# ruotianluo/ImageCaptioning.pytorch

Hardware: AMD Instinct MI355X
Metric: captions/sec/node (UpDown SCST, bs10xsample_n5, 36x2048 feats) (higher is better)
Workload: dtype f32; 1 GPU; UpDown SCST (BASELINE configs[2]): per-GPU batch 10 x train_sample_n 5, 36x2048 bottom-up feats, R=E=1000 A=512, vocab 9487, seq_len 20, references packed+cooked + greedy baseline + CIDEr-D + RewardCriterion + BPTT + clip 0.1 + Adam; rotating_batches=4, global_batch=10, seq_len=20, parallelism=dp1 (flat fp32 gradient, no collective)

## Files before the change

imagecaptioning/pytorch_amd/_lib.py:

```python
import ctypes as C
import os

import torch

HERE = os.path.dirname(os.path.abspath(__file__))
LIB_PATH = os.environ.get('CAPMI_LIB') or os.path.join(HERE, 'libcapmi.so')
MAX_SEG = 4
MAX_BCOL = 3
EINVAL = -1

c_f = C.c_void_p


class GemmSeg(C.Structure):
    _fields_ = [('A', c_f), ('B', c_f), ('lda', C.c_int), ('ldb', C.c_int), ('K', C.c_int), ('a_row_div', C.c_int)]


class GemmDesc(C.Structure):
    _fields_ = [('seg', GemmSeg * MAX_SEG), ('nseg', C.c_int), ('a_layout', C.c_int), ('b_layout', C.c_int),
                ('M', C.c_int), ('N', C.c_int), ('C', c_f), ('ldc', C.c_int), ('bias', c_f), ('bias2', c_f),
                ('row_bias', c_f), ('row_bias_div', C.c_int), ('mul_mask', c_f), ('relu', C.c_int),
                ('accumulate', C.c_int), ('partial', c_f), ('partial_capacity', C.c_int64), ('splits', C.c_int),
                ('defer_reduce', C.c_int), ('splits_used', C.c_int), ('a_planes', c_f * MAX_SEG), ('addend', c_f),
                ('allow_wide_deferred', C.c_int), ('n_bcol', C.c_int), ('bcol_B', c_f * MAX_BCOL), ('bcol_ldb', C.c_int * MAX_BCOL),
# ... 5 lines not shown
                ('alive', c_f)]


class UpDownWeights(C.Structure):
    _fields_ = [(k, c_f) for k in (
        'embed', 'att_w_ih', 'att_w_hh', 'att_b_ih', 'att_b_hh', 'lang_w_ih', 'lang_w_hh', 'lang_b_ih', 'lang_b_hh',
        'h2att_w', 'h2att_b', 'alpha_w', 'alpha_b', 'logit_w', 'logit_b')]


class UpDownRollout(C.Structure):
    _fields_ = ([(k, C.c_int) for k in ('B', 'n', 'N', 'K', 'A', 'R', 'E', 'V1', 'B_feat')] + [('row_img', c_f)] +
                [(k, C.c_int) for k in ('T', 'L')] +
                [(k, c_f) for k in ('fc', 'att', 'p_att', 'att_mask', 'drop_xt', 'drop_out')] +
                [('mode', C.c_int), ('row_mode', c_f), ('temperature', C.c_float), ('gumbel', c_f),
                 ('seed', C.c_uint64), ('forced', c_f), ('forced_ld', C.c_int), ('teacher', C.c_int)] +
                [(k, c_f) for k in ('h_att', 'c_att', 'h_lang', 'c_lang', 'xt', 'it_all', 'gates_att', 'gates_lang',
                                    'att_h', 'alpha', 'ctx', 'h_drop', 'seq', 'seq_logp', 'sel_logp', 'live',
                                    'fc_gates', 'logits', 'it', 'unfinished', 'partial')] +
                [('partial_capacity', C.c_int64), ('top_k', C.c_int), ('top_p', C.c_float), ('ss_mode', c_f),
                 ('planes', c_f), ('planes_bytes', C.c_int64), ('early_exit', C.c_int), ('early_exit_from', C.c_int),
                 ('alive_host', c_f), ('steps_run', C.c_int), ('pre_partial', c_f), ('pre_capacity', C.c_int64), ('raw_logits', C.c_int)])


class SampleFilter(C.Structure):
    _fields_ = [('top_k', C.c_int), ('top_p', C.c_float)]


class UpDownGrads(C.Structure):
    _fields_ = [(k, c_f) for k in (
        'embed', 'att_w_ih', 'att_w_hh', 'att_b_ih', 'att_b_hh', 'lang_w_ih', 'lang_w_hh', 'lang_b_ih', 'lang_b_hh',
        'h2att_w', 'h2att_b', 'alpha_w', 'alpha_b', 'logit_w', 'logit_b', 'd_fc', 'd_att', 'd_p_att')]


class SparseLogpGrad(C.Structure):
    _fields_ = [('g_sel', c_f), ('g_sum', c_f), ('tok', c_f), ('tok_ld', C.c_int), ('raw', C.c_int), ('scale', c_f)]


class MaskDesc(C.Structure):
    _fields_ = [('mask', c_f), ('count', C.c_int64), ('offset', C.c_uint64), ('row_len', C.c_int), ('rows', C.c_int),
                ('keep_from', C.c_int)]


class ReduceItem(C.Structure):
    _fields_ = [('partial', c_f), ('C', c_f), ('bias', c_f), ('splits', C.c_int32), ('M', C.c_int32), ('N', C.c_int32),
                ('ldc', C.c_int32), ('accumulate', C.c_int32), ('reserved', C.c_int32)]

# ... 124 lines not shown

class Ensemble(C.Structure):
    _fields_ = ([(k, C.c_int) for k in ('M', 'rows', 'V1', 'ld_in', 'ld_out')] + [('in', c_f * ENSEMBLE_MAX),
                ('w', C.c_float * ENSEMBLE_MAX), ('out', c_f)])


class Ppo(C.Structure):
    _fields_ = ([(k, C.c_int) for k in ('N', 'L', 'V1', 'n', 'ld_new', 'ld_old', 'ld_grad', 'per_row')] +
                [('eps', C.c_float), ('kl_coef', C.c_float)] +
                [(k, c_f) for k in ('lp_new', 'lp_old', 'seq', 'scores', 'row_stats', 'msum', 'out', 'loss_rows', 'g_out', 'grad')])


_I, _F, _P, _U64, _I64 = C.c_int, C.c_float, C.c_void_p, C.c_uint64, C.c_int64
DECODE_NO_REPEAT, DECODE_NO_BAD_ENDING, DECODE_BLOCK_TRIGRAMS = 1, 2, 4
SELECT_RAW = 256

SIGNATURES = {
    'capmi_version': [],
    'capmi_arch': [],
    'capmi_gemm_f32': [C.POINTER(GemmDesc), _P],
    'capmi_planes_bytes': [_I],
    'capmi_planes_from_f32': [_P, _I, _I, _I, _P, _P],
    'capmi_updown_planes_bytes': [_I, _I],
    'capmi_updown_bwd_planes_bytes': [_I],
    'capmi_attention_fwd': [_P] * 8 + [_I] * 5 + [_P, _I, _P],
    'capmi_attention_fwd_partial': [_P, _I, _I64, _P, _P] + [_P] * 7 + [_I] * 5 + [_P, _I, _P],
    'capmi_attention_fwd_partial_pl': [_P, _I, _I64, _P, _P] + [_P] * 7 + [_I] * 5 + [_P, _I, _P, _P],
    'capmi_attention_bwd': [_P, _I] + [_P] * 8 + [_I] * 5 + [_P, _I, _P],
    'capmi_attention_bwd_partial': [_P, _I, _I64, _I, _P] + [_P] * 7 + [_I] * 5 + [_P, _I, _P],
    'capmi_attention_bwd_batched': [_P, _I] + [_P] * 9 + [_I] * 7 + [_P],
    'capmi_attention_bwd_batched_ws': [_P, _I] + [_P] * 9 + [_I] * 7 + [_P, _P],
    'capmi_lstm_cell_fwd': [_P, _I, _P, _P, _P, _I, _P] + [_P] * 6 + [_I, _I, _P],
    'capmi_lstm_cell_fwd_pl': [_P, _I, _P, _P, _P, _I, _P] + [_P] * 6 + [_I, _I, _P, _P, _P],
    'capmi_lstm_cell_fwd_pl2': [_P, _I, _P, _I, _P, _P, _P, _I, _P] + [_P] * 6 + [_I, _I, _P, _P, _P],
    'capmi_lstm_cell_bwd': [_P, _I, _P, _P, _I, _P, _I] + [_P] * 6 + [_I, _I, _P],
    'capmi_lstm_cell_bwd_partial_pl': [_P, _I, _P, _P, _I, _I, _I64, _P, _I, _I, _I64] + [_P] * 6 + [_I, _I, _P, _P],
    'capmi_embed_fwd_pl': [_P, _I, _P, _P, _P, _P, _I, _I, _I, _P, _P],
    'capmi_lstm_cell_bwd_partial': [_P, _I, _P, _P, _I, _I, _I64, _P, _I, _I, _I64] + [_P] * 6 + [_I, _I, _P],
    'capmi_embed_fwd': [_P, _I, _P, _P, _P, _P, _I, _I, _I, _P],
    'capmi_embed_bwd': [_P] * 5 + [_I, _I, _I, _P],
    'capmi_logsoftmax_select': [_P, _I, _I, _I, _I, _I, _P, _F, _P, _U64, _P, _I, _I, _P, _I, _P, _P, _P, _P, _P, _P],
    'capmi_logsoftmax_select_partial': [_P, _I, _I64, _P, _I, _I, _I, _I, _I, _P, _F, _P, _U64, _P, _I, _I, _P, _I, _P, _P, _P,
                                        _P, _P, _P, _P, _P],
    'capmi_logsoftmax_select_partial_gemm': [_P, _I, _I64, _P, _I, _I, _I, _I, _I, _P, _F, _P, _U64, _P, _I, _I, _P, _I, _P, _P, _P,
                                        _P, _P, _P, _P, _P, _P],
    'capmi_logsoftmax_bwd': [_P, _P, _P, _P, _I, _I, _I, _I, _P],
# ... 135 lines not shown
```

imagecaptioning/pytorch_amd/captioning/models/AttModel.py:

```python
import torch
import torch.nn as nn

from .CaptionModel import CaptionModel
from imagecaptioning.pytorch_amd import updown_engine as engine
from imagecaptioning.pytorch_amd import ops
from imagecaptioning.pytorch_amd import sparse_logp
from imagecaptioning.pytorch_amd._lib import CapmiError

from .utils import parse_sample_method, clip_len


class _RolloutFn(torch.autograd.Function):

    @staticmethod
    def forward(ctx, model, cfg, fc_feats, att_feats, att_masks, *params):
        P = dict(zip(model._param_names, [p.detach() for p in params]))
        if cfg.get('fused_greedy'):
            B = fc_feats.shape[0]
            K = clip_len(att_masks, att_feats.shape[1])
            R, A = P['fc_embed.0.weight'].shape[0], P['ctx2att.weight'].shape[0]
            dev = fc_feats.device
            pr_run = engine.Prepared()
            pr_run.fc = torch.empty(2 * B, R, dtype=torch.float32, device=dev)
            pr_run.att = torch.empty(2 * B, K, R, dtype=torch.float32, device=dev)
            pr_run.p_att = torch.empty(2 * B, K, A, dtype=torch.float32, device=dev)
            pr = engine.prepare(P, fc_feats, att_feats, att_masks, cfg.get('drop_fc'), cfg.get('drop_att'),
                                out=(pr_run.fc[:B], pr_run.att[:B], pr_run.p_att[:B]))
            engine.prepare(P, fc_feats, att_feats, att_masks, out=(pr_run.fc[B:], pr_run.att[B:], pr_run.p_att[B:]))
            pr_run.att_masks = None if pr.att_masks is None else torch.cat([pr.att_masks, pr.att_masks], 0)
            extra = dict(row_img=cfg['row_img'], B_grad=B)
        else:
            pr = engine.prepare(P, fc_feats, att_feats, att_masks, cfg.get('drop_fc'), cfg.get('drop_att'))
            pr_run, extra = pr, {}
        ro = engine.Rollout(P, pr_run, n=cfg['n'], T=cfg['T'], L=cfg['L'], mode=cfg['mode'],
                            temperature=cfg.get('temperature', 1.0), drop_xt=cfg.get('drop_xt'),
                            drop_out=cfg.get('drop_out'), gumbel=cfg.get('gumbel'), seed=cfg.get('seed', 0),
                            forced=cfg.get('forced'), teacher=cfg.get('teacher', False), row_mode=cfg.get('row_mode'),
                            top_k=cfg.get('top_k', 0), top_p=cfg.get('top_p', 0.0), ss_mode=cfg.get('ss_mode'),
                            raw_logits=cfg.get('raw_logits', False), **extra)
        seq, seq_logp = ro.run()
        ctx.model, ctx.ro, ctx.pr, ctx.P = model, ro, pr, P
        ctx.sink = sink = cfg.get('_sink')
        if sink is not None:
            sink.sel, sink.seq = ro.sel_logp, ro.seq
        ctx.set_materialize_grads(False)
        ctx.mark_non_differentiable(seq)
        model._last_rollout = ro
        return seq, seq_logp.detach()

    @staticmethod
    def backward(ctx, _g_seq, g_logp):
        model, ro, pr, P = ctx.model, ctx.ro, ctx.pr, ctx.P
# ... 259 lines not shown
```

imagecaptioning/pytorch_amd/csrc/gemm_f32.hip:

```cpp
#include "host_common.h"
#include "profile.h"
#include "gemm_common.h"
#include <atomic>
#include <stdio.h>
#include <stdlib.h>
#include <hip/hip_ext.h>

using namespace capmi_gemm;

namespace {

template <int ROWS, bool KC>
__device__ __forceinline__ void g2r(f32x4 (&r)[ROWS * BK / 4 / NT], const float *__restrict__ src, int ld,
                                    int row0, int nrows, int k0, int K, int row_div, int vec) {
    constexpr int NV = ROWS * BK / 4 / NT;
#pragma unroll
    for (int p = 0; p < NV; ++p) {
        const int idx = p * NT + threadIdx.x;
        f32x4 v = {0.f, 0.f, 0.f, 0.f};
        if (KC) {
            const int rr = idx / (BK / 4);
            const int kq = (idx % (BK / 4)) * 4;
            const int row = row0 + rr;
            const int k = k0 + kq;
// ... 203 lines not shown
            for (int s0 = 0; s0 < a.splits; s0 += 8) {
                float tv[8];
#pragma unroll
                for (int u = 0; u < 8; ++u) tv[u] = (s0 + u < a.splits) ? pp[(size_t)(s0 + u) * MN] : 0.f;
#pragma unroll
                for (int u = 0; u < 8; ++u) v += tv[u];
            }
            if (a.bias) v += a.bias[col];
            if (a.bias2) v += a.bias2[col];
            if (a.row_bias) v += a.row_bias[(size_t)(row / a.row_bias_div) * a.N + col];
            if (a.relu) v = fmaxf(v, 0.f);
            if (a.mul_mask) v *= a.mul_mask[(size_t)row * a.N + col];
            if (a.accumulate) v += a.addend[(size_t)row * a.ldc + col];
            a.C[(size_t)row * a.ldc + col] = v;
        }
    }
    if (threadIdx.x == 0) __hip_atomic_store(ticket, 0, __ATOMIC_RELAXED, __HIP_MEMORY_SCOPE_AGENT);
}

template <bool VEC>
__global__ void splitk_reduce_kernel(const float *__restrict__ partial, int splits, float *__restrict__ C, int ldc,
                                     int M, int N, const float *bias, const float *bias2, const float *row_bias,
                                     int row_bias_div, const float *mul_mask, int relu, int accumulate,
                                     const float *__restrict__ addend) {
    const size_t total = (size_t)M * N;
    if (VEC) {
        const unsigned quads = (unsigned)(total >> 2), nq = (unsigned)N >> 2;
        for (unsigned q = blockIdx.x * blockDim.x + threadIdx.x; q < quads; q += gridDim.x * blockDim.x) {
            const unsigned row = q / nq, col = (q - row * nq) * 4;
            const size_t i = (size_t)q * 4;
            f32x4 v = {0.f, 0.f, 0.f, 0.f};
            for (int s0 = 0; s0 < splits; s0 += 8) {
                f32x4 tv[8];
#pragma unroll
                for (int u = 0; u < 8; ++u)
                    tv[u] = (s0 + u < splits) ? *reinterpret_cast<const f32x4 *>(partial + (size_t)(s0 + u) * total + i) : f32x4{0.f, 0.f, 0.f, 0.f};
#pragma unroll
                for (int u = 0; u < 8; ++u) v += tv[u];
            }
            if (bias) v += *reinterpret_cast<const f32x4 *>(bias + col);
            if (bias2) v += *reinterpret_cast<const f32x4 *>(bias2 + col);
            if (row_bias) v += *reinterpret_cast<const f32x4 *>(row_bias + (size_t)(row / row_bias_div) * N + col);
            if (relu) { v[0] = fmaxf(v[0], 0.f); v[1] = fmaxf(v[1], 0.f); v[2] = fmaxf(v[2], 0.f); v[3] = fmaxf(v[3], 0.f); }
            if (mul_mask) v *= *reinterpret_cast<const f32x4 *>(mul_mask + i);
            if (accumulate) v += *reinterpret_cast<const f32x4 *>(addend + (size_t)row * ldc + col);
            *reinterpret_cast<f32x4 *>(C + (size_t)row * ldc + col) = v;
        }
        return;
    }
    for (size_t i = (size_t)blockIdx.x * blockDim.x + threadIdx.x; i < total; i += (size_t)gridDim.x * blockDim.x) {
        const int row = (int)(i / N), col = (int)(i % N);
        float v = 0.f;
        for (int s0 = 0; s0 < splits; s0 += 8) {
            float tv[8];
#pragma unroll
            for (int u = 0; u < 8; ++u) tv[u] = (s0 + u < splits) ? partial[(size_t)(s0 + u) * total + i] : 0.f;
#pragma unroll
            for (int u = 0; u < 8; ++u) v += tv[u];
        }
        if (bias) v += bias[col];
        if (bias2) v += bias2[col];
        if (row_bias) v += row_bias[(size_t)(row / row_bias_div) * N + col];
        if (relu) v = fmaxf(v, 0.f);
        if (mul_mask) v *= mul_mask[i];
        float *o = C + (size_t)row * ldc + col;
        if (accumulate) v += addend[(size_t)row * ldc + col];
        *o = v;
    }
}

__global__ __launch_bounds__(256) void splitk_reduce_batch_kernel(const capmi_reduce_item *__restrict__ items) {
    const capmi_reduce_item it = items[blockIdx.y];
    const size_t total = (size_t)it.M * it.N;
    const bool vec = it.N % 4 == 0 && it.ldc % 4 == 0 && ((reinterpret_cast<uintptr_t>(it.partial) | reinterpret_cast<uintptr_t>(it.C)) & 15) == 0 &&
                     (!it.bias || (reinterpret_cast<uintptr_t>(it.bias) & 15) == 0);
    if (vec) {
        const size_t quads = total / 4;
        for (size_t q = (size_t)blockIdx.x * blockDim.x + threadIdx.x; q < quads; q += (size_t)gridDim.x * blockDim.x) {
            const size_t i = q * 4;
            const int row = (int)(i / it.N), col = (int)(i % it.N);
            f32x4 v = {0.f, 0.f, 0.f, 0.f};
            for (int s0 = 0; s0 < it.splits; s0 += 4) {
                f32x4 tv[4];
#pragma unroll
                for (int u = 0; u < 4; ++u)
                    tv[u] = (s0 + u < it.splits) ? *reinterpret_cast<const f32x4 *>(it.partial + (size_t)(s0 + u) * total + i)
// ... 24 lines not shown
};
template <typename K>
void launch_one(K kernel, dim3 grid, hipStream_t st, const KArgs &a, const ProfInfo &pi) {
    hipEvent_t e0, e1;
    if (capmi_prof::take_events(pi.cls, &e0, &e1, pi.bytes, pi.flops))
        hipExtLaunchKernelGGL(kernel, grid, dim3(NT), 0, st, e0, e1, 0, a);
    else
        hipLaunchKernelGGL(kernel, grid, dim3(NT), 0, st, a);
}
template <int BM, int BN, int WM, int WN, int PF>
int launch_cfg(const KArgs &a, int al, int bl, dim3 grid, hipStream_t st, const ProfInfo &pi) {
    if (al == 0 && bl == 0) launch_one(gemm_kernel<BM, BN, WM, WN, true, true, PF>, grid, st, a, pi);
    else if (al == 0 && bl == 1) launch_one(gemm_kernel<BM, BN, WM, WN, true, false, PF>, grid, st, a, pi);
    else if (al == 1 && bl == 1) launch_one(gemm_kernel<BM, BN, WM, WN, false, false, PF>, grid, st, a, pi);
    else launch_one(gemm_kernel<BM, BN, WM, WN, false, true, PF>, grid, st, a, pi);
    CAPMI_CHECK_LAUNCH();
    return 0;
}

}

static int splitk_reduce_addend(const float *partial, int splits, float *C, int ldc, int M, int N, const float *bias, const float *bias2,
                                const float *row_bias, int row_bias_div, const float *mul_mask, int relu, int accumulate,
                                const float *addend, void *stream) {
    if (!partial || !C || splits < 1 || M <= 0 || N <= 0) return CAPMI_EINVAL;
    const size_t total = (size_t)M * N;
    const float *ad = addend ? addend : C;
    const bool vec = N % 4 == 0 && ldc % 4 == 0 && total < (1ull << 32) &&
                     ((reinterpret_cast<uintptr_t>(partial) | reinterpret_cast<uintptr_t>(C) | reinterpret_cast<uintptr_t>(bias) |
                       reinterpret_cast<uintptr_t>(bias2) | reinterpret_cast<uintptr_t>(row_bias) | reinterpret_cast<uintptr_t>(mul_mask) |
                       reinterpret_cast<uintptr_t>(ad)) & 15) == 0;
    const size_t work = vec ? total / 4 : total;
    int blocks = (int)((work + 255) / 256);
    if (blocks > 2048) blocks = 2048;
    if (vec)
        hipLaunchKernelGGL(splitk_reduce_kernel<true>, dim3(blocks), dim3(256), 0, (hipStream_t)stream, partial, splits, C, ldc, M, N, bias,
                           bias2, row_bias, row_bias_div > 0 ? row_bias_div : 1, mul_mask, relu, accumulate, ad);
    else
        hipLaunchKernelGGL(splitk_reduce_kernel<false>, dim3(blocks), dim3(256), 0, (hipStream_t)stream, partial, splits, C, ldc, M, N, bias,
                           bias2, row_bias, row_bias_div > 0 ? row_bias_div : 1, mul_mask, relu, accumulate, ad);
    CAPMI_CHECK_LAUNCH();
    return 0;
}

extern "C" int capmi_splitk_reduce(const float *partial, int splits, float *C, int ldc, int M, int N,
                                   const float *bias, const float *bias2, const float *row_bias, int row_bias_div,
                                   const float *mul_mask, int relu, int accumulate, void *stream) {
    return splitk_reduce_addend(partial, splits, C, ldc, M, N, bias, bias2, row_bias, row_bias_div, mul_mask, relu, accumulate, nullptr,
                                stream);
}

extern "C" int capmi_splitk_reduce_batch(const capmi_reduce_item *items, int n_items, void *stream) {
    if (!items || n_items <= 0) return CAPMI_EINVAL;
    hipLaunchKernelGGL(splitk_reduce_batch_kernel, dim3(64, n_items), dim3(256), 0, (hipStream_t)stream, items);
    CAPMI_CHECK_LAUNCH();
    return 0;
}

static std::atomic<int> g_wide_deferred{0};

extern "C" int capmi_gemm_set_policy(int allow_wide_deferred) {
    return g_wide_deferred.exchange(allow_wide_deferred ? 1 : 0);
}

extern "C" int capmi_gemm_f32(capmi_gemm_desc *d, void *stream) {
    if (!d || d->nseg < 1 || d->nseg > CAPMI_MAX_SEG || d->M <= 0 || d->N <= 0 || !d->C) return CAPMI_EINVAL;
    if (d->a_layout < 0 || d->a_layout > 1 || d->b_layout < 0 || d->b_layout > 1) return CAPMI_EINVAL;
    KArgs a{};
    a.nseg = d->nseg;
    static_assert(CAPMI_MAX_BCOL == MAX_BCOL, "column segments of the descriptor and of the kernel arguments");
    if (d->n_bcol < 0 || d->n_bcol > MAX_BCOL) return CAPMI_EINVAL;
    if (d->n_bcol > 0) {
        if (d->nseg != 1 || d->b_layout != 1) return CAPMI_EINVAL;
        int ncol = 0, blk = 0;
        for (int i = 0; i < d->n_bcol; ++i) {
            if (!d->bcol_B[i] || d->bcol_n[i] <= 0 || d->bcol_n[i] % 4 || d->bcol_ldb[i] % 4 || d->bcol_ldb[i] < d->bcol_n[i] ||
                !aligned16(d->bcol_B[i]))
                return CAPMI_EINVAL;
            a.bcol[i] = BCol{d->bcol_B[i], d->bcol_ldb[i], d->bcol_n[i], blk, ncol};
            ncol += d->bcol_n[i];
            blk += (d->bcol_n[i] + 127) / 128;
        }
        if (ncol != d->N) return CAPMI_EINVAL;
        a.nbcol = d->n_bcol;
    }
    int tiles = 0;
    for (int s = 0; s < d->nseg; ++s) {
        capmi_gemm_seg g = d->seg[s];
        if (a.nbcol) { g.B = a.bcol[0].B; g.ldb = a.bcol[0].ldb; }
        if (g.K <= 0) return CAPMI_EINVAL;
// ... 18 lines not shown
    a.ablate = env_ablate;
    a.M = d->M; a.N = d->N; a.C = d->C; a.ldc = d->ldc;
    a.bias = d->bias; a.bias2 = d->bias2; a.row_bias = d->row_bias;
    a.row_bias_div = d->row_bias_div > 0 ? d->row_bias_div : 1;
    a.mul_mask = d->mul_mask; a.relu = d->relu; a.accumulate = d->accumulate;
    a.addend = d->addend ? d->addend : d->C;
    const int64_t slab_cap = d->partial ? d->partial_capacity - CAPMI_WS_COUNTER_FLOATS : 0;
    a.partial = d->partial ? d->partial + CAPMI_WS_COUNTER_FLOATS : nullptr;
    a.counters = reinterpret_cast<int *>(d->partial);
    hipStream_t st = (hipStream_t)stream;
    double ksum = 0, abytes = 0;
    for (int s = 0; s < d->nseg; ++s) {
        ksum += d->seg[s].K;
        abytes += (double)d->seg[s].K * ((double)d->M / a.seg[s].a_row_div);
    }
    const double bytes = 4.0 * (abytes + ksum * d->N + (double)d->M * d->N);
    const double flops = 2.0 * d->M * (double)d->N * ksum;
    int pcls = (d->M <= 64 && d->a_layout == 0) ? (d->b_layout == 0 ? CAPMI_PROF_GEMM_DECODE : CAPMI_PROF_GEMM_BPTT)
                                                 : CAPMI_PROF_GEMM_FAT;
    if (pcls == CAPMI_PROF_GEMM_DECODE && bytes >= 24e6) pcls = CAPMI_PROF_GEMM_DECODE_STREAM;

    static const int env_path = capmi::research("CAPMI_GEMM_PATH", 0);
    static const int env_blocks = capmi::research("CAPMI_GEMM_BLOCKS", 512);
    bool ares_ok = d->a_layout == 0 && d->M <= 64 && BK == 32;
    for (int s = 0; s < d->nseg && ares_ok; ++s)
        ares_ok = a.seg[s].vecA && (a.seg[s].K % 4 == 0) && (d->b_layout == 1 || a.seg[s].vecB);
    static const int env_lc = capmi::knob("CAPMI_LC", 1);
    {
        bool lc_ok = env_lc && env_path != 3 && ares_ok && d->M <= 64;
        for (int s = 0; s < d->nseg && lc_ok; ++s)
            lc_ok = d->a_planes[s] != nullptr && a.seg[s].a_row_div == 1 && a.seg[s].vecB;
        if (lc_ok && d->b_layout == 1) lc_ok = d->N % 4 == 0 && d->N >= 4;
        if (lc_ok) {
            static const int env_ab = capmi::research("CAPMI_ARES_BLOCKS", 256);
            static const int env_opt = capmi::research("CAPMI_LC_OPT", 1);
            const int want = d->splits > 0 ? ((d->N + 127) / 128) * d->splits : env_ab;
            int splits = 0;
            a.sl = lc_plan(d->N, tiles, want, &splits);
            const bool partial = splits > 1 || d->defer_reduce;
            if (!partial || (d->partial && (int64_t)splits * d->M * d->N <= slab_cap)) {
                a.splits = splits;
                a.to_partial = partial ? 1 : 0;
                a.self_reduce = 0;
                a.ablate = env_opt;
                d->splits_used = splits;
                int rc = launch_lc(a, d->b_layout, st, pcls, bytes, flops);
                if (rc) return rc;
                if (splits > 1 && !d->defer_reduce)
                    return splitk_reduce_addend(a.partial, splits, d->C, d->ldc, d->M, d->N, d->bias, d->bias2, d->row_bias,
                                               a.row_bias_div, d->mul_mask, d->relu, d->accumulate, d->addend, stream);
                return 0;
            }
        }
    }
    if (a.nbcol) return CAPMI_EINVAL;
    if (env_path != 3 && ares_ok) {
        static const int env_ab = capmi::research("CAPMI_ARES_BLOCKS", 256);
        static const int env_ax3 = capmi::knob("CAPMI_ARES_X3", 1);
        int use_x3 = env_ax3;
        const int want = d->splits > 0 ? ((d->N + 127) / 128) * d->splits : env_ab;
        int splits = 0;
        int ts_cap = ares_ts_cap(d->M, use_x3);
        int ts_max = ares_plan(d->N, tiles, want, ts_cap, &splits);
        if (use_x3 && ((d->N + 127) / 128) * splits > want) {
            const int nblk = (d->N + 127) / 128;
            int splits2 = 0;
            const int ts2 = ares_plan(d->N, tiles, 2 * want, 3, &splits2);
            if (nblk * splits2 <= 2 * want && (int64_t)splits2 * d->M * d->N <= slab_cap) {
                ts_cap = 3; ts_max = ts2; splits = splits2;
            } else {
                int splits32 = 0;
                const int ts32 = ares_plan(d->N, tiles, want, ares_ts_cap(d->M, 0), &splits32);
                if (nblk * splits32 <= want) {
                    use_x3 = 0; ts_cap = ares_ts_cap(d->M, 0); ts_max = ts32; splits = splits32;
                }
            }
        }
        if ((splits > 1 || d->defer_reduce) && (int64_t)splits * d->M * d->N > slab_cap) ts_max = 99;
        if (ts_max <= ts_cap) {
            a.splits = splits;
            a.to_partial = (splits > 1 || d->defer_reduce) ? 1 : 0;
            a.self_reduce = 0;
            static const int env_aopt = capmi::research("CAPMI_ARES_OPT", 2);
            a.ablate = env_aopt;
            if (a.to_partial && (!d->partial || (int64_t)splits * d->M * d->N > slab_cap)) return CAPMI_EINVAL;
            d->splits_used = splits;
            int rc = launch_ares(a, d->b_layout, ts_max, use_x3, st, pcls, bytes, flops);
            if (rc) return rc;
            if (splits > 1 && !d->defer_reduce)
                return splitk_reduce_addend(a.partial, splits, d->C, d->ldc, d->M, d->N, d->bias, d->bias2, d->row_bias,
                                           a.row_bias_div, d->mul_mask, d->relu, d->accumulate, d->addend, stream);
            return 0;
        }
    }

    static const int env_cfg = capmi::research("CAPMI_GEMM_CFG", 1);
    int BM, BN;
    (void)env_cfg;
    if (d->M <= 32) { BM = 32; BN = 128; }
    else if (d->M <= 64 || (long long)d->M * d->N < 256LL * 1024) {
        BM = 64;
        BN = (d->b_layout == 0 && tiles >= 64 && d->N >= 1024) ? 128 : 64;
        if (env_cfg == 64 || env_cfg == 128) BN = env_cfg;
    } else { BM = 128; BN = 128; }
    const int gm = (d->M + BM - 1) / BM, gn = (d->N + BN - 1) / BN;
    static const int env_x3 = capmi::knob("CAPMI_GEMM_X3", 1);
    bool x3_ok = env_x3 && BM == 128 && BN == 128 && BK == 32 &&
                 (d->a_layout == 0 || d->M % 4 == 0) && (d->b_layout == 0 || d->N % 4 == 0);
    for (int s = 0; s < d->nseg && x3_ok; ++s)
        x3_ok = a.seg[s].a_row_div == 1 && a.seg[s].vecA && a.seg[s].vecB && a.seg[s].K % 4 == 0 &&
                (uint64_t)(d->a_layout == 0 ? d->M : 1) * (uint64_t)a.seg[s].lda * 4 < (1ull << 32) &&
                (uint64_t)(d->b_layout == 0 ? d->N : 1) * (uint64_t)a.seg[s].ldb * 4 < (1ull << 32);
    int splits = d->splits;
    static const int env_tile = capmi::knob("CAPMI_X3_TILE", 0);
    static const int env_wcost = capmi::research("CAPMI_X3W_COST", 165);
    static const int env_swap = capmi::knob("CAPMI_X3_SWAP", 1);
    int tiling = 0;
    const int gmw = (d->M + 255) / 256, gnw = (d->N + 255) / 256;
    if (x3_ok) {
        double best = 1e30;
        int best_sp = 1;
        const int sp_lo = splits > 0 ? splits : 1, sp_hi = splits > 0 ? splits : 16;
        for (int w = 0; w < 3; ++w) {
            if ((w == 0 && env_tile == 256) || (w >= 1 && env_tile == 128)) continue;
            if (w == 1 && env_tile != 256 && gmw < 4) continue;
            if (w == 1 && env_tile != 256 && d->defer_reduce && !d->allow_wide_deferred && !g_wide_deferred.load(std::memory_order_relaxed)) continue;
            if (w == 2 && (env_swap == 0 || d->a_layout != 0 || gnw < 4 || gmw >= 4)) continue;
            const int out_tiles = w == 0 ? gm * gn : w == 1 ? gmw * gn : gnw * gm;
            const double step = w ? env_wcost / 100.0 : 1.0;
            for (int sp = sp_lo; sp <= sp_hi && sp <= tiles; ++sp) {
                if (splits == 0 && sp > 1 && (!d->partial || (int64_t)sp * d->M * d->N > slab_cap)) break;
                const double rounds = (double)((out_tiles * sp + 255) / 256);
                const double slab_us = sp > 1 ? (2.0 * sp + 1.0) * d->M * (double)d->N * 4.0 / 4.0e6 : 0.0;
                const double cost = rounds * ((tiles + sp - 1) / sp) * step + slab_us / 1.5;
                if (cost < best) { best = cost; best_sp = sp; tiling = w; }
            }
        }
        if (splits == 0) splits = best_sp;
    } else if (splits == 0) {
        const int blocks = gm * gn;
        splits = 1;
        if (blocks < env_blocks * 3 / 4 && d->partial) {
            splits = (env_blocks + blocks - 1) / blocks;
            if (splits > tiles / 4) splits = tiles / 4;
            if (splits > 64) splits = 64;
            if (splits < 1) splits = 1;
            while (splits > 1 && (int64_t)splits * d->M * d->N > slab_cap) --splits;
        }
    }
    if (splits > tiles) splits = tiles;
    a.splits = splits;
    a.to_partial = (splits > 1 || d->defer_reduce) ? 1 : 0;
    static const int env_self = capmi::research("CAPMI_GEMM_SELF_REDUCE", 0);
    a.self_reduce = (env_self && splits > 1 && !d->defer_reduce && gn * gm <= CAPMI_WS_COUNTER_FLOATS) ? 1 : 0;
    if (x3_ok) a.self_reduce = 0;
    if (a.to_partial && (!d->partial || (int64_t)splits * d->M * d->N > slab_cap)) return CAPMI_EINVAL;
    d->splits_used = splits;
    static const int env_log = capmi::knob("CAPMI_GEMM_LOG", 0);
    if (env_log)
        fprintf(stderr, "capmi_gemm M=%d N=%d tiles=%d al=%d bl=%d x3=%d wide=%d splits=%d defer=%d acc=%d\n", d->M, d->N, tiles,
                d->a_layout, d->b_layout, (int)x3_ok, x3_ok ? tiling : 0, splits, d->defer_reduce, d->accumulate);
    dim3 grid(gn, gm, splits);
    const ProfInfo pi{pcls, bytes, flops};
    int rc;
    if (x3_ok && tiling == 1) rc = launch_x3w(a, d->a_layout, d->b_layout, dim3(gn, gmw, splits), st, pcls, bytes, flops);
    else if (x3_ok && tiling == 2) {
        KArgs t = a;
        for (int s2 = 0; s2 < CAPMI_MAX_SEG; ++s2) {
            t.seg[s2].A = a.seg[s2].B; t.seg[s2].B = a.seg[s2].A;
            t.seg[s2].lda = a.seg[s2].ldb; t.seg[s2].ldb = a.seg[s2].lda;
            t.seg[s2].vecA = a.seg[s2].vecB; t.seg[s2].vecB = a.seg[s2].vecA;
            t.seg[s2].Apl = nullptr;
        }
        t.M = a.N; t.N = a.M;
        t.transposed = 1;
        rc = launch_x3w(t, d->b_layout, d->a_layout, dim3(gm, gnw, splits), st, pcls, bytes, flops);
    } else if (x3_ok) rc = launch_x3(a, d->a_layout, d->b_layout, grid, st, pcls, bytes, flops);
    else if (BM == 32 && BN == 128) rc = launch_cfg<32, 128, 1, 4, 3>(a, d->a_layout, d->b_layout, grid, st, pi);
    else if (BM == 64 && BN == 64) rc = launch_cfg<64, 64, 2, 2, 3>(a, d->a_layout, d->b_layout, grid, st, pi);
        else if (BM == 64 && BN == 128) rc = launch_cfg<64, 128, 1, 4, 2>(a, d->a_layout, d->b_layout, grid, st, pi);
    else rc = launch_cfg<128, 128, 2, 2, 2>(a, d->a_layout, d->b_layout, grid, st, pi);
    if (rc) return rc;
    if (splits > 1 && !d->defer_reduce && !a.self_reduce)
        return splitk_reduce_addend(a.partial, splits, d->C, d->ldc, d->M, d->N, d->bias, d->bias2, d->row_bias,
                                   a.row_bias_div, d->mul_mask, d->relu, d->accumulate, d->addend, stream);
    return 0;
}

extern "C" int capmi_gemm_group_tn(capmi_group_gemm *items, int n, float *slabs, int64_t slab_floats, void *stream) {
    if (!items || n <= 0) return CAPMI_EINVAL;
    hipStream_t st = (hipStream_t)stream;
    static const int env_group = capmi::knob("CAPMI_GEMM_GROUP", 1);
    constexpr int TILE = 256 * 128;
    int order[1024], n_ok = 0, rest[1024], n_rest = 0;
    if (n > 1024) return CAPMI_EINVAL;
    for (int i = 0; i < n; ++i) {
        capmi_group_gemm &g = items[i];
        if (!g.A || !g.B || !g.C || g.K <= 0 || g.M <= 0 || g.N <= 0) return CAPMI_EINVAL;
        const bool ok = env_group && BK == 32 && g.M % 4 == 0 && g.N % 4 == 0 && g.lda % 4 == 0 && g.ldb % 4 == 0 &&
                        g.ldc % 4 == 0 && aligned16(g.A) && aligned16(g.B) && aligned16(g.C) && aligned16(g.colsum) &&
                        (uint64_t)g.lda * 16 * 4 + (uint64_t)g.M * 4 < (1ull << 32) && (uint64_t)g.ldb * 16 * 4 + (uint64_t)g.N * 4 < (1ull << 32);
        if (ok) order[n_ok++] = i;
        else rest[n_rest++] = i;
    }
    for (int i = 1; i < n_ok; ++i) {
        const int v = order[i], kv = (items[v].K + BK - 1) / BK;
        int j = i - 1;
        while (j >= 0 && (items[order[j]].K + BK - 1) / BK < kv) { order[j + 1] = order[j]; --j; }
        order[j + 1] = v;
// ... 75 lines not shown
```

imagecaptioning/pytorch_amd/updown_engine.py:

```python
import ctypes as C
import os
import math

import torch

from . import _lib, ops
from .ops import clip_len
from ._lib import lib, ptr, check, stream_ptr

_f32 = torch.float32

PARAM_KEYS = ('embed.0.weight', 'fc_embed.0.weight', 'fc_embed.0.bias', 'att_embed.0.weight', 'att_embed.0.bias',
              'ctx2att.weight', 'ctx2att.bias', 'core.att_lstm.weight_ih', 'core.att_lstm.weight_hh',
              'core.att_lstm.bias_ih', 'core.att_lstm.bias_hh', 'core.lang_lstm.weight_ih', 'core.lang_lstm.weight_hh',
              'core.lang_lstm.bias_ih', 'core.lang_lstm.bias_hh', 'core.attention.h2att.weight',
              'core.attention.h2att.bias', 'core.attention.alpha_net.weight', 'core.attention.alpha_net.bias',
              'logit.weight', 'logit.bias')

_W_FIELDS = (('embed', 'embed.0.weight'), ('att_w_ih', 'core.att_lstm.weight_ih'), ('att_w_hh', 'core.att_lstm.weight_hh'),
             ('att_b_ih', 'core.att_lstm.bias_ih'), ('att_b_hh', 'core.att_lstm.bias_hh'),
             ('lang_w_ih', 'core.lang_lstm.weight_ih'), ('lang_w_hh', 'core.lang_lstm.weight_hh'),
             ('lang_b_ih', 'core.lang_lstm.bias_ih'), ('lang_b_hh', 'core.lang_lstm.bias_hh'),
             ('h2att_w', 'core.attention.h2att.weight'), ('h2att_b', 'core.attention.h2att.bias'),
             ('alpha_w', 'core.attention.alpha_net.weight'), ('alpha_b', 'core.attention.alpha_net.bias'),
# ... 22 lines not shown
        att_masks = att_masks[:, :max_len].contiguous().float()
        if drop_att is not None:
            drop_att = drop_att[:, :max_len].contiguous()
    K = att_feats.shape[1]
    pr = Prepared()
    pr.K = K
    pr.fc_in, pr.att_in, pr.drop_fc = fc_feats.contiguous(), att_feats.contiguous(), drop_fc
    o_fc, o_att, o_patt = out if out is not None else (None, None, None)
    pr.fc = ops.linear(pr.fc_in, P['fc_embed.0.weight'], P['fc_embed.0.bias'], relu=True, mul_mask=drop_fc, ws=ws, out=o_fc)
    R = pr.fc.shape[1]
    att_mask_full = drop_att
    if att_masks is not None:
        m = att_masks.unsqueeze(-1).expand(B, K, R)
        att_mask_full = (m if drop_att is None else m * drop_att).contiguous()
    pr.drop_att = att_mask_full
    att2d = ops.linear(pr.att_in.view(B * K, -1), P['att_embed.0.weight'], P['att_embed.0.bias'], relu=True,
                       mul_mask=None if att_mask_full is None else att_mask_full.view(B * K, R), ws=ws,
                       out=None if o_att is None else o_att.view(B * K, R))
    pr.att = att2d.view(B, K, R)
    pr.p_att = ops.linear(att2d, P['ctx2att.weight'], P['ctx2att.bias'], ws=ws,
                          out=None if o_patt is None else o_patt.view(B * K, -1)).view(B, K, -1)
    pr.att_masks = att_masks
    return pr


def prepare_backward(P, pr, d_fc, d_att, d_p_att, grads, ws=None):
    B, K, R = pr.att.shape
    A = pr.p_att.shape[2]
    dp = d_p_att.view(B * K, A)
    att2d = pr.att.view(B * K, R)
    group = [] if os.environ.get('CAPMI_PREP_GROUP', '1') != '0' else None

    def dw(dy, x, wname, bname):
        if group is not None and grads[bname].data_ptr() % 16 == 0:
            group.append((dy, x, grads[wname], False, None, 0, grads[bname]))
        else:
            ops.matmul_tn(dy, x, out=grads[wname], ws=ws)
            ops.colsum(dy, out=grads[bname])
    dw(dp, att2d, 'ctx2att.weight', 'ctx2att.bias')
    d_att_total = d_att.view(B * K, R)
    ops.gemm([(dp, A, P['ctx2att.weight'], R, A, 1)], B * K, R, d_att_total, a_layout=0, b_layout=1, accumulate=True, ws=ws)
    d_pre = _relu_drop_bwd(d_att_total, att2d, None if pr.drop_att is None else pr.drop_att.view(B * K, R))
    dw(d_pre, pr.att_in.view(B * K, -1), 'att_embed.0.weight', 'att_embed.0.bias')
    d_pre_fc = _relu_drop_bwd(d_fc, pr.fc, pr.drop_fc)
    dw(d_pre_fc, pr.fc_in, 'fc_embed.0.weight', 'fc_embed.0.bias')
    if group:
# ... 148 lines not shown
```

include/capmi.h:

```cpp
#ifndef CAPMI_H
#define CAPMI_H

#include <stdint.h>

#ifdef __cplusplus
extern "C" {
#endif

#define CAPMI_EINVAL (-1)
#define CAPMI_MAX_SEG 4
#define CAPMI_MAX_BCOL 3
#define CAPMI_WS_COUNTER_FLOATS 16384

int capmi_version(void);
const char *capmi_arch(void);

typedef struct capmi_gemm_seg {
    const float *A;
    const float *B;
    int lda;
    int ldb;
    int K;
    int a_row_div;
} capmi_gemm_seg;
// ... 289 lines not shown
    float *logits;
    int64_t *it;
    uint8_t *unfinished;
    float *partial;
    int64_t partial_capacity;
    int top_k;
    float top_p;
    const uint8_t *ss_mode;
    void *planes;
    int64_t planes_bytes;
    int early_exit;
    int early_exit_from;
    int32_t *alive_host;
    int steps_run;
    float *pre_partial;
    int64_t pre_capacity;
    int raw_logits;
} capmi_updown_rollout;

int64_t capmi_updown_planes_bytes(int R, int E);

int capmi_updown_rollout_fwd(const capmi_updown_weights *w, capmi_updown_rollout *r, void *stream);

typedef struct capmi_updown_grads {
    float *embed;
    float *att_w_ih, *att_w_hh, *att_b_ih, *att_b_hh;
    float *lang_w_ih, *lang_w_hh, *lang_b_ih, *lang_b_hh;
    float *h2att_w, *h2att_b;
    float *alpha_w, *alpha_b;
    float *logit_w, *logit_b;
    float *d_fc;
    float *d_att;
    float *d_p_att;
} capmi_updown_grads;

typedef struct capmi_updown_bwd_scratch {
    float *dlogits;
    float *d_hdrop;
    float *dg_att;
    float *dg_lang;
    float *d_x2;
    float *d_e_all;
    float *d_att_h_all;
    float *dh_att_attn;
    float *d_x1;
    float *dc_att, *dc_lang;
// ... 373 lines not shown
```

Baseline: 12610 captions/s.

## Compute dropout and clean prepare embeddings in one GEMM with dual-output epilogue

Fused greedy SCST previously ran the prepare stage twice: once with dropout masks for the sampled rollout and once without for the greedy baseline. A new C entry point now runs each embedding GEMM once. Its split-K reduce epilogue writes two outputs, one with the dropout mask and one with only the attention mask, and ctx2att runs as a single stacked GEMM over both halves when the row count exceeds 64. This halves the large att_embed GEMM work and removes Python launches, but it forces the result through the partial-slab reduce path even when no split is used, and it adds tiling planning based on a separate planned row count.

```diff
diff --git a/imagecaptioning/pytorch_amd/_lib.py b/imagecaptioning/pytorch_amd/_lib.py
--- a/imagecaptioning/pytorch_amd/_lib.py
+++ b/imagecaptioning/pytorch_amd/_lib.py
@@ -51,6 +51,13 @@
                  ('alive_host', c_f), ('steps_run', C.c_int), ('pre_partial', c_f), ('pre_capacity', C.c_int64), ('raw_logits', C.c_int)])
 
 
+class PreparePair(C.Structure):
+    _fields_ = ([(k, C.c_int) for k in ('B', 'K', 'F_fc', 'F_att', 'R', 'A')] +
+                [(k, c_f) for k in ('fc_in', 'att_in', 'fc_w', 'fc_b', 'att_w', 'att_b', 'ctx_w', 'ctx_b', 'fc_mask0', 'fc_mask1',
+                                    'att_mask0', 'att_mask1', 'fc_out', 'att_out', 'p_att_out', 'partial')] +
+                [('partial_capacity', C.c_int64)])
+
+
 class SampleFilter(C.Structure):
     _fields_ = [('top_k', C.c_int), ('top_p', C.c_float)]
 
@@ -221,6 +228,7 @@
     'capmi_planes_bytes': [_I],
     'capmi_planes_from_f32': [_P, _I, _I, _I, _P, _P],
     'capmi_updown_planes_bytes': [_I, _I],
+    'capmi_updown_prepare_pair': [C.POINTER(PreparePair), _P],
     'capmi_updown_bwd_planes_bytes': [_I],
     'capmi_attention_fwd': [_P] * 8 + [_I] * 5 + [_P, _I, _P],
     'capmi_attention_fwd_partial': [_P, _I, _I64, _P, _P] + [_P] * 7 + [_I] * 5 + [_P, _I, _P],
diff --git a/imagecaptioning/pytorch_amd/captioning/models/AttModel.py b/imagecaptioning/pytorch_amd/captioning/models/AttModel.py
--- a/imagecaptioning/pytorch_amd/captioning/models/AttModel.py
+++ b/imagecaptioning/pytorch_amd/captioning/models/AttModel.py
@@ -1,3 +1,5 @@
+import os
+
 import torch
 import torch.nn as nn
 
@@ -17,17 +19,20 @@
         P = dict(zip(model._param_names, [p.detach() for p in params]))
         if cfg.get('fused_greedy'):
             B = fc_feats.shape[0]
-            K = clip_len(att_masks, att_feats.shape[1])
-            R, A = P['fc_embed.0.weight'].shape[0], P['ctx2att.weight'].shape[0]
-            dev = fc_feats.device
-            pr_run = engine.Prepared()
-            pr_run.fc = torch.empty(2 * B, R, dtype=torch.float32, device=dev)
-            pr_run.att = torch.empty(2 * B, K, R, dtype=torch.float32, device=dev)
-            pr_run.p_att = torch.empty(2 * B, K, A, dtype=torch.float32, device=dev)
-            pr = engine.prepare(P, fc_feats, att_feats, att_masks, cfg.get('drop_fc'), cfg.get('drop_att'),
-                                out=(pr_run.fc[:B], pr_run.att[:B], pr_run.p_att[:B]))
-            engine.prepare(P, fc_feats, att_feats, att_masks, out=(pr_run.fc[B:], pr_run.att[B:], pr_run.p_att[B:]))
-            pr_run.att_masks = None if pr.att_masks is None else torch.cat([pr.att_masks, pr.att_masks], 0)
+            if os.environ.get('CAPMI_PREP_PAIR', '1') != '0':
+                pr, pr_run = engine.prepare_pair(P, fc_feats, att_feats, att_masks, cfg.get('drop_fc'), cfg.get('drop_att'))
+            else:
+                K = clip_len(att_masks, att_feats.shape[1])
+                R, A = P['fc_embed.0.weight'].shape[0], P['ctx2att.weight'].shape[0]
+                dev = fc_feats.device
+                pr_run = engine.Prepared()
+                pr_run.fc = torch.empty(2 * B, R, dtype=torch.float32, device=dev)
+                pr_run.att = torch.empty(2 * B, K, R, dtype=torch.float32, device=dev)
+                pr_run.p_att = torch.empty(2 * B, K, A, dtype=torch.float32, device=dev)
+                pr = engine.prepare(P, fc_feats, att_feats, att_masks, cfg.get('drop_fc'), cfg.get('drop_att'),
+                                    out=(pr_run.fc[:B], pr_run.att[:B], pr_run.p_att[:B]))
+                engine.prepare(P, fc_feats, att_feats, att_masks, out=(pr_run.fc[B:], pr_run.att[B:], pr_run.p_att[B:]))
+                pr_run.att_masks = None if pr.att_masks is None else torch.cat([pr.att_masks, pr.att_masks], 0)
             extra = dict(row_img=cfg['row_img'], B_grad=B)
         else:
             pr = engine.prepare(P, fc_feats, att_feats, att_masks, cfg.get('drop_fc'), cfg.get('drop_att'))
diff --git a/imagecaptioning/pytorch_amd/csrc/gemm_f32.hip b/imagecaptioning/pytorch_amd/csrc/gemm_f32.hip
--- a/imagecaptioning/pytorch_amd/csrc/gemm_f32.hip
+++ b/imagecaptioning/pytorch_amd/csrc/gemm_f32.hip
@@ -249,7 +249,7 @@
 __global__ void splitk_reduce_kernel(const float *__restrict__ partial, int splits, float *__restrict__ C, int ldc,
                                      int M, int N, const float *bias, const float *bias2, const float *row_bias,
                                      int row_bias_div, const float *mul_mask, int relu, int accumulate,
-                                     const float *__restrict__ addend) {
+                                     const float *__restrict__ addend, float *__restrict__ C2, const float *mul_mask2) {
     const size_t total = (size_t)M * N;
     if (VEC) {
         const unsigned quads = (unsigned)(total >> 2), nq = (unsigned)N >> 2;
@@ -269,6 +269,11 @@
             if (bias2) v += *reinterpret_cast<const f32x4 *>(bias2 + col);
             if (row_bias) v += *reinterpret_cast<const f32x4 *>(row_bias + (size_t)(row / row_bias_div) * N + col);
             if (relu) { v[0] = fmaxf(v[0], 0.f); v[1] = fmaxf(v[1], 0.f); v[2] = fmaxf(v[2], 0.f); v[3] = fmaxf(v[3], 0.f); }
+            if (C2) {
+                f32x4 w = v;
+                if (mul_mask2) w *= *reinterpret_cast<const f32x4 *>(mul_mask2 + i);
+                *reinterpret_cast<f32x4 *>(C2 + (size_t)row * ldc + col) = w;
+            }
             if (mul_mask) v *= *reinterpret_cast<const f32x4 *>(mul_mask + i);
             if (accumulate) v += *reinterpret_cast<const f32x4 *>(addend + (size_t)row * ldc + col);
             *reinterpret_cast<f32x4 *>(C + (size_t)row * ldc + col) = v;
@@ -289,6 +294,7 @@
         if (bias2) v += bias2[col];
         if (row_bias) v += row_bias[(size_t)(row / row_bias_div) * N + col];
         if (relu) v = fmaxf(v, 0.f);
+        if (C2) C2[(size_t)row * ldc + col] = mul_mask2 ? v * mul_mask2[i] : v;
         if (mul_mask) v *= mul_mask[i];
         float *o = C + (size_t)row * ldc + col;
         if (accumulate) v += addend[(size_t)row * ldc + col];
@@ -359,23 +365,24 @@
 
 static int splitk_reduce_addend(const float *partial, int splits, float *C, int ldc, int M, int N, const float *bias, const float *bias2,
                                 const float *row_bias, int row_bias_div, const float *mul_mask, int relu, int accumulate,
-                                const float *addend, void *stream) {
+                                const float *addend, void *stream, float *C2 = nullptr, const float *mul_mask2 = nullptr) {
     if (!partial || !C || splits < 1 || M <= 0 || N <= 0) return CAPMI_EINVAL;
+    if (C2 ? accumulate != 0 : mul_mask2 != nullptr) return CAPMI_EINVAL;
     const size_t total = (size_t)M * N;
     const float *ad = addend ? addend : C;
     const bool vec = N % 4 == 0 && ldc % 4 == 0 && total < (1ull << 32) &&
                      ((reinterpret_cast<uintptr_t>(partial) | reinterpret_cast<uintptr_t>(C) | reinterpret_cast<uintptr_t>(bias) |
                        reinterpret_cast<uintptr_t>(bias2) | reinterpret_cast<uintptr_t>(row_bias) | reinterpret_cast<uintptr_t>(mul_mask) |
-                       reinterpret_cast<uintptr_t>(ad)) & 15) == 0;
+                       reinterpret_cast<uintptr_t>(ad) | reinterpret_cast<uintptr_t>(C2) | reinterpret_cast<uintptr_t>(mul_mask2)) & 15) == 0;
     const size_t work = vec ? total / 4 : total;
     int blocks = (int)((work + 255) / 256);
     if (blocks > 2048) blocks = 2048;
     if (vec)
         hipLaunchKernelGGL(splitk_reduce_kernel<true>, dim3(blocks), dim3(256), 0, (hipStream_t)stream, partial, splits, C, ldc, M, N, bias,
-                           bias2, row_bias, row_bias_div > 0 ? row_bias_div : 1, mul_mask, relu, accumulate, ad);
+                           bias2, row_bias, row_bias_div > 0 ? row_bias_div : 1, mul_mask, relu, accumulate, ad, C2, mul_mask2);
     else
         hipLaunchKernelGGL(splitk_reduce_kernel<false>, dim3(blocks), dim3(256), 0, (hipStream_t)stream, partial, splits, C, ldc, M, N, bias,
-                           bias2, row_bias, row_bias_div > 0 ? row_bias_div : 1, mul_mask, relu, accumulate, ad);
+                           bias2, row_bias, row_bias_div > 0 ? row_bias_div : 1, mul_mask, relu, accumulate, ad, C2, mul_mask2);
     CAPMI_CHECK_LAUNCH();
     return 0;
 }
@@ -400,9 +407,27 @@
     return g_wide_deferred.exchange(allow_wide_deferred ? 1 : 0);
 }
 
-extern "C" int capmi_gemm_f32(capmi_gemm_desc *d, void *stream) {
+struct PairOut {
+    float *C2;
+    const float *mul_mask2;
+    int plan_M;
+};
+
+static int gemm_f32_impl(capmi_gemm_desc *d, void *stream, const PairOut *x) {
     if (!d || d->nseg < 1 || d->nseg > CAPMI_MAX_SEG || d->M <= 0 || d->N <= 0 || !d->C) return CAPMI_EINVAL;
     if (d->a_layout < 0 || d->a_layout > 1 || d->b_layout < 0 || d->b_layout > 1) return CAPMI_EINVAL;
+    const int pM = (x && x->plan_M > 0) ? x->plan_M : d->M;
+    float *const C2 = x ? x->C2 : nullptr;
+    const float *const mask2 = x ? x->mul_mask2 : nullptr;
+    const bool two = C2 != nullptr;
+    if (two && (d->accumulate || d->defer_reduce || d->n_bcol || !d->partial)) return CAPMI_EINVAL;
+    if (pM <= 64 && d->M > 64) return CAPMI_EINVAL;
+    const bool to_slabs = d->defer_reduce || two;
+    auto finish = [&](const float *partial, int splits, int row_bias_div) -> int {
+        if (d->defer_reduce || (splits <= 1 && !two)) return 0;
+        return splitk_reduce_addend(partial, splits, d->C, d->ldc, d->M, d->N, d->bias, d->bias2, d->row_bias, row_bias_div, d->mul_mask,
+                                    d->relu, d->accumulate, d->addend, stream, C2, mask2);
+    };
     KArgs a{};
     a.nseg = d->nseg;
     static_assert(CAPMI_MAX_BCOL == MAX_BCOL, "column segments of the descriptor and of the kernel arguments");
@@ -467,7 +492,7 @@
 
     static const int env_path = capmi::research("CAPMI_GEMM_PATH", 0);
     static const int env_blocks = capmi::research("CAPMI_GEMM_BLOCKS", 512);
-    bool ares_ok = d->a_layout == 0 && d->M <= 64 && BK == 32;
+    bool ares_ok = d->a_layout == 0 && pM <= 64 && BK == 32;
     for (int s = 0; s < d->nseg && ares_ok; ++s)
         ares_ok = a.seg[s].vecA && (a.seg[s].K % 4 == 0) && (d->b_layout == 1 || a.seg[s].vecB);
     static const int env_lc = capmi::knob("CAPMI_LC", 1);
@@ -482,7 +507,7 @@
             const int want = d->splits > 0 ? ((d->N + 127) / 128) * d->splits : env_ab;
             int splits = 0;
             a.sl = lc_plan(d->N, tiles, want, &splits);
-            const bool partial = splits > 1 || d->defer_reduce;
+            const bool partial = splits > 1 || to_slabs;
             if (!partial || (d->partial && (int64_t)splits * d->M * d->N <= slab_cap)) {
                 a.splits = splits;
                 a.to_partial = partial ? 1 : 0;
@@ -491,10 +516,7 @@
                 d->splits_used = splits;
                 int rc = launch_lc(a, d->b_layout, st, pcls, bytes, flops);
                 if (rc) return rc;
-                if (splits > 1 && !d->defer_reduce)
-                    return splitk_reduce_addend(a.partial, splits, d->C, d->ldc, d->M, d->N, d->bias, d->bias2, d->row_bias,
-                                               a.row_bias_div, d->mul_mask, d->relu, d->accumulate, d->addend, stream);
-                return 0;
+                return finish(a.partial, splits, a.row_bias_div);
             }
         }
     }
@@ -521,10 +543,10 @@
                 }
             }
         }
-        if ((splits > 1 || d->defer_reduce) && (int64_t)splits * d->M * d->N > slab_cap) ts_max = 99;
+        if ((splits > 1 || to_slabs) && (int64_t)splits * d->M * d->N > slab_cap) ts_max = 99;
         if (ts_max <= ts_cap) {
             a.splits = splits;
-            a.to_partial = (splits > 1 || d->defer_reduce) ? 1 : 0;
+            a.to_partial = (splits > 1 || to_slabs) ? 1 : 0;
             a.self_reduce = 0;
             static const int env_aopt = capmi::research("CAPMI_ARES_OPT", 2);
             a.ablate = env_aopt;
@@ -532,23 +554,21 @@
             d->splits_used = splits;
             int rc = launch_ares(a, d->b_layout, ts_max, use_x3, st, pcls, bytes, flops);
             if (rc) return rc;
-            if (splits > 1 && !d->defer_reduce)
-                return splitk_reduce_addend(a.partial, splits, d->C, d->ldc, d->M, d->N, d->bias, d->bias2, d->row_bias,
-                                           a.row_bias_div, d->mul_mask, d->relu, d->accumulate, d->addend, stream);
-            return 0;
+            return finish(a.partial, splits, a.row_bias_div);
         }
     }
 
     static const int env_cfg = capmi::research("CAPMI_GEMM_CFG", 1);
     int BM, BN;
     (void)env_cfg;
-    if (d->M <= 32) { BM = 32; BN = 128; }
-    else if (d->M <= 64 || (long long)d->M * d->N < 256LL * 1024) {
+    if (pM <= 32) { BM = 32; BN = 128; }
+    else if (pM <= 64 || (long long)pM * d->N < 256LL * 1024) {
         BM = 64;
         BN = (d->b_layout == 0 && tiles >= 64 && d->N >= 1024) ? 128 : 64;
         if (env_cfg == 64 || env_cfg == 128) BN = env_cfg;
     } else { BM = 128; BN = 128; }
     const int gm = (d->M + BM - 1) / BM, gn = (d->N + BN - 1) / BN;
+    const int pgm = (pM + BM - 1) / BM, pgmw = (pM + 255) / 256;
     static const int env_x3 = capmi::knob("CAPMI_GEMM_X3", 1);
     bool x3_ok = env_x3 && BM == 128 && BN == 128 && BK == 32 &&
                  (d->a_layout == 0 || d->M % 4 == 0) && (d->b_layout == 0 || d->N % 4 == 0);
@@ -568,37 +588,37 @@
         const int sp_lo = splits > 0 ? splits : 1, sp_hi = splits > 0 ? splits : 16;
         for (int w = 0; w < 3; ++w) {
             if ((w == 0 && env_tile == 256) || (w >= 1 && env_tile == 128)) continue;
-            if (w == 1 && env_tile != 256 && gmw < 4) continue;
+            if (w == 1 && env_tile != 256 && pgmw < 4) continue;
             if (w == 1 && env_tile != 256 && d->defer_reduce && !d->allow_wide_deferred && !g_wide_deferred.load(std::memory_order_relaxed)) continue;
-            if (w == 2 && (env_swap == 0 || d->a_layout != 0 || gnw < 4 || gmw >= 4)) continue;
-            const int out_tiles = w == 0 ? gm * gn : w == 1 ? gmw * gn : gnw * gm;
+            if (w == 2 && (env_swap == 0 || d->a_layout != 0 || gnw < 4 || pgmw >= 4)) continue;
+            const int out_tiles = w == 0 ? pgm * gn : w == 1 ? pgmw * gn : gnw * pgm;
             const double step = w ? env_wcost / 100.0 : 1.0;
             for (int sp = sp_lo; sp <= sp_hi && sp <= tiles; ++sp) {
-                if (splits == 0 && sp > 1 && (!d->partial || (int64_t)sp * d->M * d->N > slab_cap)) break;
+                if (splits == 0 && sp > 1 && (!d->partial || (int64_t)sp * pM * d->N > slab_cap)) break;
                 const double rounds = (double)((out_tiles * sp + 255) / 256);
-                const double slab_us = sp > 1 ? (2.0 * sp + 1.0) * d->M * (double)d->N * 4.0 / 4.0e6 : 0.0;
+                const double slab_us = sp > 1 ? (2.0 * sp + 1.0) * pM * (double)d->N * 4.0 / 4.0e6 : 0.0;
                 const double cost = rounds * ((tiles + sp - 1) / sp) * step + slab_us / 1.5;
                 if (cost < best) { best = cost; best_sp = sp; tiling = w; }
             }
         }
         if (splits == 0) splits = best_sp;
     } else if (splits == 0) {
-        const int blocks = gm * gn;
+        const int blocks = pgm * gn;
         splits = 1;
         if (blocks < env_blocks * 3 / 4 && d->partial) {
             splits = (env_blocks + blocks - 1) / blocks;
             if (splits > tiles / 4) splits = tiles / 4;
             if (splits > 64) splits = 64;
             if (splits < 1) splits = 1;
-            while (splits > 1 && (int64_t)splits * d->M * d->N > slab_cap) --splits;
+            while (splits > 1 && (int64_t)splits * pM * d->N > slab_cap) --splits;
         }
     }
     if (splits > tiles) splits = tiles;
     a.splits = splits;
-    a.to_partial = (splits > 1 || d->defer_reduce) ? 1 : 0;
+    a.to_partial = (splits > 1 || to_slabs) ? 1 : 0;
     static const int env_self = capmi::research("CAPMI_GEMM_SELF_REDUCE", 0);
     a.self_reduce = (env_self && splits > 1 && !d->defer_reduce && gn * gm <= CAPMI_WS_COUNTER_FLOATS) ? 1 : 0;
-    if (x3_ok) a.self_reduce = 0;
+    if (x3_ok || two) a.self_reduce = 0;
     if (a.to_partial && (!d->partial || (int64_t)splits * d->M * d->N > slab_cap)) return CAPMI_EINVAL;
     d->splits_used = splits;
     static const int env_log = capmi::knob("CAPMI_GEMM_LOG", 0);
@@ -626,10 +646,39 @@
         else if (BM == 64 && BN == 128) rc = launch_cfg<64, 128, 1, 4, 2>(a, d->a_layout, d->b_layout, grid, st, pi);
     else rc = launch_cfg<128, 128, 2, 2, 2>(a, d->a_layout, d->b_layout, grid, st, pi);
     if (rc) return rc;
-    if (splits > 1 && !d->defer_reduce && !a.self_reduce)
-        return splitk_reduce_addend(a.partial, splits, d->C, d->ldc, d->M, d->N, d->bias, d->bias2, d->row_bias,
-                                   a.row_bias_div, d->mul_mask, d->relu, d->accumulate, d->addend, stream);
-    return 0;
+    if (a.self_reduce) return 0;
+    return finish(a.partial, splits, a.row_bias_div);
+}
+
+extern "C" int capmi_gemm_f32(capmi_gemm_desc *d, void *stream) { return gemm_f32_impl(d, stream, nullptr); }
+
+extern "C" int capmi_updown_prepare_pair(const capmi_prepare_pair *p, void *stream) {
+    if (!p || p->B <= 0 || p->K <= 0 || p->F_fc <= 0 || p->F_att <= 0 || p->R <= 0 || p->A <= 0) return CAPMI_EINVAL;
+    if (!p->fc_in || !p->att_in || !p->fc_w || !p->att_w || !p->ctx_w || !p->fc_out || !p->att_out || !p->p_att_out || !p->partial)
+        return CAPMI_EINVAL;
+    const int B = p->B, R = p->R, A = p->A;
+    const int64_t rows = (int64_t)B * p->K;
+    if (2 * rows * (R > A ? R : A) >= (1ll << 31)) return CAPMI_EINVAL;
+    const int M = (int)rows;
+    auto linear = [&](const float *X, int F, const float *W, const float *b, int m, int n, float *out, const float *mask, int relu,
+                      const PairOut &x) -> int {
+        capmi_gemm_desc d{};
+        d.nseg = 1;
+        d.seg[0].A = X; d.seg[0].B = W; d.seg[0].lda = F; d.seg[0].ldb = F; d.seg[0].K = F; d.seg[0].a_row_div = 1;
+        d.M = m; d.N = n; d.C = out; d.ldc = n;
+        d.bias = b; d.row_bias_div = 1; d.mul_mask = mask; d.relu = relu;
+        d.partial = p->partial; d.partial_capacity = p->partial_capacity;
+        return gemm_f32_impl(&d, stream, &x);
+    };
+    int rc = linear(p->fc_in, p->F_fc, p->fc_w, p->fc_b, B, R, p->fc_out, p->fc_mask0, 1, PairOut{p->fc_out + (size_t)B * R, p->fc_mask1, 0});
+    if (rc) return rc;
+    rc = linear(p->att_in, p->F_att, p->att_w, p->att_b, M, R, p->att_out, p->att_mask0, 1,
+                PairOut{p->att_out + (size_t)M * R, p->att_mask1, 0});
+    if (rc) return rc;
+    if (M > 64) return linear(p->att_out, R, p->ctx_w, p->ctx_b, 2 * M, A, p->p_att_out, nullptr, 0, PairOut{nullptr, nullptr, M});
+    rc = linear(p->att_out, R, p->ctx_w, p->ctx_b, M, A, p->p_att_out, nullptr, 0, PairOut{nullptr, nullptr, 0});
+    if (rc) return rc;
+    return linear(p->att_out + (size_t)M * R, R, p->ctx_w, p->ctx_b, M, A, p->p_att_out + (size_t)M * A, nullptr, 0, PairOut{nullptr, nullptr, 0});
 }
 
 extern "C" int capmi_gemm_group_tn(capmi_group_gemm *items, int n, float *slabs, int64_t slab_floats, void *stream) {
diff --git a/imagecaptioning/pytorch_amd/updown_engine.py b/imagecaptioning/pytorch_amd/updown_engine.py
--- a/imagecaptioning/pytorch_amd/updown_engine.py
+++ b/imagecaptioning/pytorch_amd/updown_engine.py
@@ -68,6 +68,52 @@
                           out=None if o_patt is None else o_patt.view(B * K, -1)).view(B, K, -1)
     pr.att_masks = att_masks
     return pr
+
+
+def prepare_pair(P, fc_feats, att_feats, att_masks=None, drop_fc=None, drop_att=None, ws=None):
+    B = fc_feats.shape[0]
+    if att_masks is not None:
+        max_len = clip_len(att_masks)
+        att_feats = att_feats[:, :max_len].contiguous()
+        att_masks = att_masks[:, :max_len].contiguous().float()
+        if drop_att is not None:
+            drop_att = drop_att[:, :max_len].contiguous()
+    K = att_feats.shape[1]
+    R, A = P['fc_embed.0.weight'].shape[0], P['ctx2att.weight'].shape[0]
+    dev = fc_feats.device
+    pr = Prepared()
+    pr.K = K
+    pr.fc_in, pr.att_in, pr.drop_fc = fc_feats.contiguous(), att_feats.contiguous(), drop_fc
+    mask0 = mask1 = drop_att
+    if att_masks is not None:
+        m = att_masks.unsqueeze(-1).expand(B, K, R)
+        mask1 = m.contiguous()
+        mask0 = mask1 if drop_att is None else (m * drop_att).contiguous()
+    elif drop_att is not None:
+        mask1 = None
+    pr.drop_att, pr.att_masks = mask0, att_masks
+    pr_run = Prepared()
+    pr_run.fc = torch.empty(2 * B, R, dtype=_f32, device=dev)
+    pr_run.att = torch.empty(2 * B, K, R, dtype=_f32, device=dev)
+    pr_run.p_att = torch.empty(2 * B, K, A, dtype=_f32, device=dev)
+    pr_run.att_masks = None if att_masks is None else torch.cat([att_masks, att_masks], 0)
+    weights = [P[k] for k in ('fc_embed.0.weight', 'fc_embed.0.bias', 'att_embed.0.weight', 'att_embed.0.bias', 'ctx2att.weight', 'ctx2att.bias')]
+    ops._chk(pr.fc_in, pr.att_in, drop_fc, mask0, mask1, *weights)
+    if pr.fc_in.shape[1] != weights[0].shape[1] or pr.att_in.shape[2] != weights[2].shape[1] or weights[4].shape[1] != R:
+        raise _lib.CapmiError('prepare_pair: feature widths %d / %d against weights %s / %s / %s' % (
+            pr.fc_in.shape[1], pr.att_in.shape[2], tuple(weights[0].shape), tuple(weights[2].shape), tuple(weights[4].shape)))
+    if ws is None:
+        ws = ops.default_workspace(dev)
+    d = _lib.PreparePair()
+    d.B, d.K, d.F_fc, d.F_att, d.R, d.A = B, K, pr.fc_in.shape[1], pr.att_in.shape[2], R, A
+    d.fc_in, d.att_in = ptr(pr.fc_in), ptr(pr.att_in)
+    d.fc_w, d.fc_b, d.att_w, d.att_b, d.ctx_w, d.ctx_b = (ptr(w) for w in weights)
+    d.fc_mask0, d.fc_mask1, d.att_mask0, d.att_mask1 = ptr(drop_fc), None, ptr(mask0), ptr(mask1)
+    d.fc_out, d.att_out, d.p_att_out = ptr(pr_run.fc), ptr(pr_run.att), ptr(pr_run.p_att)
+    d.partial, d.partial_capacity = ws.buf.data_ptr(), ws.capacity
+    check(lib.capmi_updown_prepare_pair(C.byref(d), stream_ptr()), 'capmi_updown_prepare_pair')
+    pr.fc, pr.att, pr.p_att = pr_run.fc[:B], pr_run.att[:B], pr_run.p_att[:B]
+    return pr, pr_run
 
 
 def prepare_backward(P, pr, d_fc, d_att, d_p_att, grads, ws=None):
diff --git a/include/capmi.h b/include/capmi.h
--- a/include/capmi.h
+++ b/include/capmi.h
@@ -335,6 +335,23 @@
 
 int capmi_updown_rollout_fwd(const capmi_updown_weights *w, capmi_updown_rollout *r, void *stream);
 
+typedef struct capmi_prepare_pair {
+    int B, K, F_fc, F_att, R, A;
+    const float *fc_in;
+    const float *att_in;
+    const float *fc_w, *fc_b;
+    const float *att_w, *att_b;
+    const float *ctx_w, *ctx_b;
+    const float *fc_mask0, *fc_mask1;
+    const float *att_mask0, *att_mask1;
+    float *fc_out;
+    float *att_out;
+    float *p_att_out;
+    float *partial;
+    int64_t partial_capacity;
+} capmi_prepare_pair;
+int capmi_updown_prepare_pair(const capmi_prepare_pair *p, void *stream);
+
 typedef struct capmi_updown_grads {
     float *embed;
     float *att_w_ih, *att_w_hh, *att_b_ih, *att_b_hh;
```

Measured after the change: 12700 captions/s (median of 2 runs). Within noise of the previous version (+0.7%).
